# BGI-Qingdao/HAST

Hardware: AMD Instinct MI355X
Metric: classified read-bp/sec at k=21, 150bp reads, 200M unique-mers/hap (higher is better)
Workload: dtype u64; 1 GPU; C3 human-trio scale: 200M+200M synthetic 21-mers, 10M barcodes, 150bp reads; k=21, read_len=150, keys_per_hap=200000000, barcodes=10000000, batch_reads=48000000, reads_total=5760000000, minimizer=16, keys=random, collective=none (D2H of counters in timed region), resident_batches=12

## Files before the change

### hast_amd/binding.py

```python
import ctypes as C
import os
import subprocess

import numpy as np

_HERE = os.path.dirname(os.path.abspath(__file__))
_LIB = None

u8p, u32p, u64p, vp = C.POINTER(C.c_uint8), C.POINTER(C.c_uint32), C.POINTER(C.c_uint64), C.c_void_p

STATUS = {0: "OK", 1: "INVALID", 2: "NO_DEVICE", 3: "HIP", 4: "OOM", 5: "TABLE_FULL", 6: "FORMAT", 7: "RCCL", 8: "IO", 9: "UNSUPPORTED"}


class SynthParams(C.Structure):
    _fields_ = [("seed_k", C.c_uint64), ("seed_r", C.c_uint64), ("seed_b", C.c_uint64),
                ("n_keys_per_hap", C.c_uint64), ("n_barcodes", C.c_uint32), ("read_len", C.c_uint32),
                ("k", C.c_uint32), ("reserved", C.c_uint32)]


class KcSynth(C.Structure):
    _fields_ = [("seed", C.c_uint64), ("genome_len", C.c_uint64), ("read_len", C.c_uint32), ("snp_per_1024", C.c_uint32),
                ("err_per_4096", C.c_uint32), ("n_per_4096", C.c_uint32)]


# ... 64 lines not shown
    "hast_dev_alloc": (C.c_int, [vp, C.c_size_t, C.POINTER(vp)]),
    "hast_dev_free": (C.c_int, [vp, vp]),
    "hast_memcpy_h2d": (C.c_int, [vp, vp, vp, C.c_size_t]),
    "hast_memcpy_d2h": (C.c_int, [vp, vp, vp, C.c_size_t]),
    "hast_memset_d": (C.c_int, [vp, vp, C.c_int, C.c_size_t, vp]),
    "hast_table_reserve": (C.c_int, [vp, C.c_uint64, C.c_double]),
    "hast_table_insert_text": (C.c_int, [vp, C.c_int, C.c_char_p, C.c_size_t, u64p]),
    "hast_table_insert_text_file": (C.c_int, [vp, C.c_int, C.c_char_p, u64p]),
    "hast_ctx_set_text_check": (C.c_int, [vp, C.c_int]),
    "hast_table_insert_keys": (C.c_int, [vp, C.c_int, vp, C.c_size_t]),
    "hast_table_insert_keys_device": (C.c_int, [vp, C.c_int, vp, C.c_size_t, vp]),
    "hast_table_erase": (C.c_int, [vp, vp, C.c_size_t, vp]),
    "hast_table_sizes": (C.c_int, [vp, u64p, u64p]),
    "hast_table_lookup": (C.c_int, [vp, vp, C.c_size_t, vp]),
    "hast_table_save": (C.c_int, [vp, C.c_char_p]),
    "hast_table_load": (C.c_int, [vp, C.c_char_p, C.c_double]),
    "hast_table_file_info": (C.c_int, [C.c_char_p, C.POINTER(C.c_int), u64p]),
    "hast_table_info": (C.c_int, [vp, u64p, u64p]),
    "hast_table_clone": (C.c_int, [vp, vp]),
    "hast_ctx_set_filter": (C.c_int, [vp, C.c_int, C.c_int, C.c_int, C.c_int]),
    "hast_filter_build": (C.c_int, [vp]),
    "hast_filter_info": (C.c_int, [vp, C.POINTER(C.c_int), C.POINTER(C.c_int), C.POINTER(C.c_int), C.POINTER(C.c_int), u64p]),
    "hast_filter_dense": (C.c_int, [vp, C.POINTER(C.c_int)]),
    "hast_filter_request_ceiling": (C.c_int, [vp, C.POINTER(C.c_double)]),
    "hast_counts_resize": (C.c_int, [vp, C.c_size_t]),
    "hast_counts_bind": (C.c_int, [vp, vp, C.c_size_t]),
    "hast_counts_zero": (C.c_int, [vp, vp]),
    "hast_counts_read": (C.c_int, [vp, vp, vp, vp, C.c_size_t]),
    "hast_counts_pack": (C.c_int, [vp, vp, C.c_size_t, vp]),
    "hast_counts_unpack": (C.c_int, [vp, vp, C.c_size_t, vp]),
    "hast_counts_add_votes": (C.c_int, [vp, vp, vp, C.c_size_t, C.c_uint32, vp]),
    "hast_counts_allreduce": (C.c_int, [C.POINTER(vp), C.c_int]),
    "hast_classify_timing": (C.c_int, [vp, C.c_int]),
    "hast_classify_times": (C.c_int, [vp, C.POINTER(C.c_float), C.POINTER(C.c_float), C.c_int, C.POINTER(C.c_int)]),
    "hast_classify_device": (C.c_int, [vp, vp, C.c_size_t, vp, C.c_uint32, vp, vp, C.c_size_t, vp]),
    "hast_classify_batch": (C.c_int, [vp, vp, vp, vp, C.c_size_t, C.c_uint32]),
    "hast_classify_perread_device": (C.c_int, [vp, vp, C.c_size_t, vp, C.c_size_t, vp, vp]),
    "hast_classify_perread": (C.c_int, [vp, vp, vp, C.c_size_t, vp]),
    "hast_batch_begin": (C.c_int, [vp, C.c_size_t, C.c_size_t, C.POINTER(vp), C.POINTER(vp), C.POINTER(vp)]),
    "hast_batch_submit": (C.c_int, [vp, C.c_size_t, C.c_uint32]),
    "hast_names_create": (C.c_int, [vp, C.c_size_t, C.POINTER(vp)]),
    "hast_names_destroy": (None, [vp]),
    "hast_fq_create": (C.c_int, [vp, C.c_size_t, C.c_int, vp, C.POINTER(vp)]),
    "hast_fq_create_ex": (C.c_int, [vp, C.c_size_t, C.c_int, vp, C.c_int, C.POINTER(vp)]),
    "hast_fq_create_striped": (C.c_int, [C.POINTER(vp), C.c_int, C.c_size_t, C.c_int, C.POINTER(vp), C.POINTER(vp)]),
    "hast_fq_create_striped_ex": (C.c_int, [C.POINTER(vp), C.c_int, C.c_size_t, C.c_int, C.POINTER(vp), C.c_int, C.POINTER(vp)]),
# ... 239 lines not shown
    def filter_build(self):
        _ck(self._lib.hast_filter_build(self._h))

    def filter_request_ceiling(self):
        r = C.c_double()
        _ck(self._lib.hast_filter_request_ceiling(self._h, C.byref(r)))
        return r.value

    def filter_info(self):
        en, m, t, kp, b = C.c_int(), C.c_int(), C.c_int(), C.c_int(), C.c_uint64()
        _ck(self._lib.hast_filter_info(self._h, C.byref(en), C.byref(m), C.byref(t), C.byref(kp), C.byref(b)))
        return bool(en.value), m.value, t.value, kp.value, b.value

    def filter_mode(self):
        en = C.c_int()
        _ck(self._lib.hast_filter_info(self._h, C.byref(en), None, None, None, None))
        return en.value

    def filter_dense(self):
        d = C.c_int()
        _ck(self._lib.hast_filter_dense(self._h, C.byref(d)))
        return bool(d.value)

    def close(self):
        if self._h:
            self._lib.hast_ctx_destroy(self._h)
            self._h = C.c_void_p()

    def __enter__(self):
        return self

    def __exit__(self, *a):
        self.close()

    def __del__(self):
        try:
            self.close()
        except Exception:
            pass

    @property
    def stream(self):
        return self._lib.hast_ctx_stream(self._h)

    def sync(self, stream=None):
        _ck(self._lib.hast_stream_sync(self._h, stream))
# ... 499 lines not shown
```

### hast_amd/csrc/classify_main.cpp

```cpp
#include <getopt.h>
#include <sys/stat.h>
#include <unistd.h>

#include <algorithm>
#include <atomic>
#include <cerrno>
#include <chrono>
#include <deque>
#include <cstdarg>
#include <cstdio>
#include <cstdlib>
#include <cstring>
#include <ctime>
#include <condition_variable>
#include <memory>
#include <mutex>
#include <string>
#include <thread>
#include <string_view>
#include <unordered_map>
#include <vector>

#include "../../include/hast.h"
#include "fq_feed.h"
// ... 1771 lines not shown
                (unsigned long long)rs.total_bases, rs.names.size(), rs.t_loaded - rs.t_start, dt, dt > 0 ? rs.total_bases / dt / 1e6 : 0.0);
    }
    if (o.stats && rs.naming.device_dict)
        stat_line("__stats_dictionary__ on=device dictionaries=%zu ids_limit=%zu ids_from_device=%zu ids_from_host=%zu merge_by_text_s=%.3f texts_merged_to_host=%zu rows_summed_by_text=%zu\n", rs.naming.groups.size(), rs.naming.host_base, rs.n_dev_names, rs.n_host_names, rs.naming.merge_s,
                  rs.naming.merged_to_host, rs.n_rows_summed);
    if (o.stats) {
        const char *nc = getenv("HAST_NAME_CACHE"), *rb = getenv("HAST_GZ_RING_BYTES"), *pg = getenv("HAST_PARK_GB");
        stat_line("__stats_sizes__ name_cache=%s gz_ring_bytes=%s park_gb=%s\n", nc ? nc : "default", rb ? rb : "default", pg ? pg : "default");
    }
    if (o.stats) stat_line("__stats_setup__ waited_for_stream_setup_s=%.3f (inside scrub_sizes_clone_s: .gz inputs opened, FASTQ streams created while the table was built)\n", rs.t_pre_waited);
    for (size_t i = 0; i < rs.ctxs.size(); i++) {
        char sw[512] = "";
        (void)hast_ctx_options(rs.ctxs[i], sw, sizeof(sw));
        if (strstr(sw, "filter_fallback"))
            fprintf(stderr, " WARN : GPU %d (context %zu) had no room for the k-mer filter and probed the table directly (%s)\n", o.devices[i], i, sw);
    }
    if (o.stats) {
        char sw[512] = "";
        (void)hast_ctx_options(rs.ctx, sw, sizeof(sw));
        stat_line("__stats_switches__ %s\n", sw[0] ? sw : "none");
        int f_on = 0, f_m = 0, f_t = 0, f_kp = 0;
        uint64_t f_bytes = 0;
        (void)hast_filter_info(rs.ctx, &f_on, &f_m, &f_t, &f_kp, &f_bytes);
        stat_line("__stats_filter__ mode=%s m=%d t=%d kp=%d bytes=%llu\n", f_on == 2 ? "exact_entries" : f_on == 1 ? "prints" : "off_table_only", f_m, f_t, f_kp,
                  (unsigned long long)f_bytes);
    }
    if (rs.hbm_thread.joinable()) {
        rs.hbm_stop = true;
        rs.hbm_thread.join();
        size_t parked = 0;
        (void)hast_dev_mem_info(rs.ctx, nullptr, nullptr, &parked);
        const size_t fm = rs.hbm_free_min.load(), tot = rs.hbm_total.load();
        if (tot) stat_line("__stats_hbm__ total_bytes=%zu free_min_bytes=%zu in_use_peak_bytes=%zu parked_bytes_at_end=%zu\n", tot, fm, tot - std::min(fm, tot), parked);
    }
    fprintf(stderr, "__END__\n");
    rs.t_printed = now_s();
}

int leave(Run &rs) {
    const Options &o = rs.o;
    const char *preload = getenv("LD_PRELOAD");
    const bool profiled = getenv("ROCP_TOOL_LIBRARIES") || (preload && strstr(preload, "rocprofiler"));
    if (!getenv("HAST_TEARDOWN") && !profiled) {
        if (o.stats) stat_phases(rs, nullptr);
        if (!o.stats_json.empty() && !write_stats_json(o.stats_json)) fprintf(stderr, "classify: cannot write %s\n", o.stats_json.c_str());
        if (fflush(stdout) != 0) die_output();
        fflush(stderr);
        _exit(0);
// ... 51 lines not shown
```

### hast_amd/csrc/hast_api.cpp

```cpp
#include <dlfcn.h>
#include <fcntl.h>
#include <sys/stat.h>
#include <unistd.h>
#include <hip/hip_runtime.h>

#include <algorithm>
#include <chrono>
#include <atomic>
#include <cstdarg>
#include <cstdio>
#include <cstdlib>
#include <cstring>
#include <functional>
#include <map>
#include <mutex>
#include <new>
#include <string>
#include <vector>

#include "../../include/hast.h"
#include "hast_common.h"
#include "hast_device.h"
#include "kc_device.h"
#include "fq_device.h"
// ... 271 lines not shown
        else c->exact_env_off = atoi(e) == 0;
    }
    if (c->exact_env_off) c->filter_exact = 0;
    else if (c->exact_env_once) c->filter_exact = 1;
    if (const char *e = getenv("HAST_COMMIT")) c->commit_mode = !strcmp(e, "atomic") ? 1 : !strcmp(e, "partition") ? 2 : 0;
    if (const char *e = getenv("HAST_PART_SPAN")) c->part_span = (uint32_t)atoi(e);
    if (const char *e = getenv("HAST_F_GEO")) c->kernel_geo = e[0] != '0';
    if (const char *e = getenv("HAST_F_RL")) c->kernel_rl = e[0] != '0';
    if (const char *e = getenv("HAST_TILE_LDS")) {
        const long v = atol(e);
        if (v >= 4096 && v <= 160 * 1024) c->tile_lds = (size_t)v;
    }
    hipDeviceProp_t prop;
    if (hipGetDeviceProperties(&prop, device) == hipSuccess) c->n_cu = prop.multiProcessorCount;
    tr("hipGetDeviceProperties");
    hast_status st = HAST_OK;
    auto bail = [&](hipError_t he, const char *what) {
        if (he != hipSuccess && st == HAST_OK) st = set_error(HAST_ERR_HIP, "%s: %s", what, hipGetErrorString(he));
    };
    bail(hipStreamCreateWithFlags(&c->stream, hipStreamNonBlocking), "hipStreamCreate");
    tr("hipStreamCreate");
    bail(dev_malloc(&c->d_err, 4 * sizeof(uint32_t)), "dev_malloc(err)");
    tr("first hipMalloc");
    bail(dev_malloc(&c->d_cnt, 8 * sizeof(unsigned long long)), "dev_malloc(cnt)");
    bail(pinned_malloc(reinterpret_cast<void **>(&c->h_errword), 64, hipHostMallocDefault), "pinned_malloc(err word)");
    if (st == HAST_OK) bail(hipMemsetAsync(c->d_err, 0, 4 * sizeof(uint32_t), c->stream), "hipMemset");
    if (st == HAST_OK) bail(hipStreamSynchronize(c->stream), "hipStreamSynchronize");
    tr("first fill + synchronize");
    for (auto &s : c->stage)
        if (st == HAST_OK) bail(hipEventCreateWithFlags(&s.done, hipEventDisableTiming), "hipEventCreate");
    tr("events");
    if (st != HAST_OK) {
        hast_ctx_destroy(c);
        return st;
    }
    *out = c;
    return HAST_OK;
}

void hast_release_parked(void) { release_parked(); }

void hast_ctx_destroy(hast_ctx *c) {
    if (!c) return;
    (void)hipSetDevice(c->device);
    if (c->stream) (void)hipStreamSynchronize(c->stream);
    release_parked();
    for (auto &s : c->stage) {
// ... 404 lines not shown
    dst->nbuckets = 0;
    dst->filter_valid = false;
    dst->m = src->m;
    const size_t bytes = table_slots(src) * sizeof(uint64_t);
    HAST_HIP_TRY(dev_malloc(&dst->d_slots, bytes));
    HAST_HIP_TRY(hipMemcpyPeerAsync(dst->d_slots, dst->device, src->d_slots, src->device, bytes, dst->stream));
    dst->nbuckets = src->nbuckets;
    if (src->filter_valid && dst->use_filter) {
        if (dst->filter_bytes != src->filter_bytes) {
            if (dst->d_filter) HAST_HIP_TRY(hipFree(dst->d_filter));
            dst->d_filter = nullptr;
            dst->filter_bytes = 0;
            if (dst->test_filter_oom || dev_malloc(&dst->d_filter, src->filter_bytes) != hipSuccess) {
                (void)hipGetLastError();
                dst->d_filter = nullptr;
                dst->use_filter = false;
                dst->filter_fallback_bytes = src->filter_bytes;
                HAST_HIP_TRY(hipStreamSynchronize(dst->stream));
                return HAST_OK;
            }
            dst->filter_bytes = src->filter_bytes;
        }
        HAST_HIP_TRY(hipMemcpyPeerAsync(dst->d_filter, dst->device, src->d_filter, src->device, src->filter_bytes, dst->stream));
        dst->fg = src->fg;
        dst->filter_m = src->filter_m;
        dst->filter_exact = src->filter_exact;
        dst->filter_t = src->filter_t;
        dst->filter_kp = src->filter_kp;
        dst->filter_valid = true;
    }
    HAST_HIP_TRY(hipStreamSynchronize(dst->stream));
    return HAST_OK;
}

hast_status hast_table_info(const hast_ctx *c, uint64_t *n_buckets, uint64_t *bytes) {
    if (!c) return set_error(HAST_ERR_INVALID, "null context");
    if (n_buckets) *n_buckets = c->nbuckets;
    if (bytes) *bytes = (uint64_t)table_slots(c) * sizeof(uint64_t);
    return HAST_OK;
}

hast_status hast_counts_resize(hast_ctx *c, size_t n) {
    if (hast_status st = use(c)) return st;
    HAST_HIP_TRY(hipStreamSynchronize(c->stream));
    if (c->counts_owned && c->d_counts) HAST_HIP_TRY(hipFree(c->d_counts));
    c->d_counts = nullptr;
// ... 199 lines not shown
    FilterGeom fg = filter_geom_for(c->k, h[0] + h[1], c->filter_m, c->filter_t, c->filter_kp, c->k == 32 ? 0 : c->filter_exact);
    size_t bytes = (size_t)filter_nblocks(fg) * 128;
    if (bytes != c->filter_bytes) {
        if (c->d_filter) HAST_HIP_TRY(hipFree(c->d_filter));
        c->d_filter = nullptr;
        c->filter_bytes = 0;
        hipError_t got = c->test_filter_oom ? hipErrorOutOfMemory : dev_malloc(&c->d_filter, bytes);
        if (got != hipSuccess && !c->filter_m && fg.m == kFilterMaxM) {
            (void)hipGetLastError();
            fg = filter_geom_for(c->k, h[0] + h[1], kFilterMaxM - 1, c->filter_t, c->filter_kp, c->k == 32 ? 0 : c->filter_exact);
            bytes = (size_t)filter_nblocks(fg) * 128;
            got = dev_malloc(&c->d_filter, bytes);
        }
        if (got != hipSuccess) {
            (void)hipGetLastError();
            c->d_filter = nullptr;
            c->use_filter = false;
            c->filter_fallback_bytes = bytes;
            return HAST_OK;
        }
        c->filter_bytes = bytes;
    }
    HAST_HIP_TRY(hipMemsetAsync(c->d_filter, 0, bytes, hs));
    HAST_HIP_TRY(launch_filter_build(c->d_slots, geom(c), c->d_filter, fg, hs));
    c->fg = fg;
    c->filter_valid = true;
    return HAST_OK;
}

static constexpr uint32_t kSegWindows = 482;
static constexpr uint32_t kLongRead = 4096;

static hast_status commit_prepare(hast_ctx *c, size_t n_reads, uint32_t max_votes, bool atomic_only, hipStream_t hs, commit::Plan *pl, bool *partitioned) {
    *partitioned = false;
    const int mode = c->commit_mode;
    if (mode == 1 || atomic_only || c->part_oom) return HAST_OK;
    *pl = commit::plan_for(n_reads, c->n_barcodes, c->part_span);
    if (!commit::usable(*pl, n_reads, max_votes, mode == 2)) return HAST_OK;
    if (c->part.bytes < pl->bytes) {
        HAST_HIP_TRY(hipStreamSynchronize(hs));
        if (c->part.d) HAST_HIP_TRY(hipFree(c->part.d));
        c->part = CommitScratch{};
        if (dev_malloc(&c->part.d, pl->bytes + pl->bytes / 8) == hipSuccess) c->part.bytes = pl->bytes + pl->bytes / 8;
        else {
            (void)hipGetLastError();
            c->part.d = nullptr;
            c->part_oom = true;
// ... 192 lines not shown
    if (hast_status st = need_table(c, 0)) return st;
    if (!c->use_filter) return HAST_OK;
    if (hast_status st = ensure_filter(c, c->stream)) return st;
    HAST_HIP_TRY(hipStreamSynchronize(c->stream));
    return HAST_OK;
}

hast_status hast_filter_info(const hast_ctx *c, int *enabled, int *m, int *t, int *kp, uint64_t *bytes) {
    if (!c) return set_error(HAST_ERR_INVALID, "null context");
    if (enabled) *enabled = !c->use_filter ? 0 : (c->filter_valid && c->fg.exact) ? 2 : 1;
    if (m) *m = c->filter_valid ? c->fg.m : 0;
    if (t) *t = c->filter_valid ? c->fg.t : 0;
    if (kp) *kp = c->filter_valid ? c->fg.kp : 0;
    if (bytes) *bytes = c->filter_valid ? c->filter_bytes : 0;
    return HAST_OK;
}

hast_status hast_filter_dense(const hast_ctx *c, int *dense) {
    if (!c || !dense) return set_error(HAST_ERR_INVALID, "null argument");
    *dense = (c->use_filter && c->filter_valid && c->fg.dense) ? 1 : 0;
    return HAST_OK;
}

hast_status hast_filter_request_ceiling(hast_ctx *c, double *requests_per_s) {
    if (hast_status st = need_table(c, 0)) return st;
    if (!requests_per_s) return set_error(HAST_ERR_INVALID, "null argument");
    if (!c->use_filter) return set_error(HAST_ERR_INVALID, "the filter is off");
    if (hast_status st = ensure_filter(c, c->stream)) return st;
    if (!c->use_filter || !c->d_filter) return set_error(HAST_ERR_INVALID, "no filter (HBM too small for it)");
    const uint64_t nblocks = filter_nblocks(c->fg);
    const int grid = c->n_cu * 8;
    const uint32_t iters = 256;
    uint32_t *d_sink = reinterpret_cast<uint32_t *>(c->d_cnt + 2);
    hipEvent_t e0 = nullptr, e1 = nullptr;
    hipError_t e = hipEventCreate(&e0);
    if (e == hipSuccess) e = hipEventCreate(&e1);
    float best = 0;
    for (int rep = 0; rep < 3 && e == hipSuccess; ++rep) {
        e = hipEventRecord(e0, c->stream);
        if (e == hipSuccess) e = launch_request_ceiling(c->d_filter, nblocks, iters, grid, d_sink, c->stream);
        if (e == hipSuccess) e = hipEventRecord(e1, c->stream);
        if (e == hipSuccess) e = hipEventSynchronize(e1);
        float ms = 0;
        if (e == hipSuccess) e = hipEventElapsedTime(&ms, e0, e1);
        if (e == hipSuccess && rep && (best == 0 || ms < best)) best = ms;
    }
// ... 335 lines not shown
```

### hast_amd/csrc/hast_common.h

```cpp
#pragma once
#include <stdint.h>

#include "tmer_level_table.h"

#if defined(__HIPCC__)
#include <hip/hip_runtime.h>
#define HAST_HD __host__ __device__ __forceinline__
#else
#define HAST_HD inline
#endif

namespace hast {

HAST_HD uint32_t base_code(uint32_t c) { return (c & 6u) >> 1; }
HAST_HD uint64_t kmer_mask(int k) { return k >= 32 ? ~0ull : (1ull << (2 * k)) - 1; }

HAST_HD uint64_t kmer_revcomp(uint64_t x, int k) {
    x ^= 0xAAAAAAAAAAAAAAAAull;
#if defined(__HIP_DEVICE_COMPILE__)
    x = __brevll(x);
    x = ((x & 0x5555555555555555ull) << 1) | ((x >> 1) & 0x5555555555555555ull);
#else
    x = ((x & 0x3333333333333333ull) << 2) | ((x >> 2) & 0x3333333333333333ull);
    x = ((x & 0x0F0F0F0F0F0F0F0Full) << 4) | ((x >> 4) & 0x0F0F0F0F0F0F0F0Full);
// ... 132 lines not shown
    return h ^ (h >> 15);
}
HAST_HD uint32_t filter_sub_of(uint32_t keyhash) { return keyhash >> 29; }
HAST_HD uint32_t filter_sub2_of(uint32_t keyhash) { return (keyhash >> 26) & 7u; }
HAST_HD uint32_t filter_print_of(uint32_t keyhash) {
    const uint32_t f = (keyhash >> 8) & 0xFFFFu;
    return f ? f : 1u;
}
HAST_HD int filter_pos_bits(const FilterGeom &g) {
    int b = 0;
    while ((1u << b) < filter_w(g)) ++b;
    return b;
}
HAST_HD bool filter_exact_fits(const FilterGeom &g) { return g.k <= 32 && g.m <= 14 && 2 * (g.k - g.m) + filter_pos_bits(g) <= 17; }
HAST_HD uint32_t filter_exact_code(uint64_t fwd, uint32_t pm, const FilterGeom &g) {
    const int rb = 2 * (g.k - g.m);
    const uint32_t rest = ((uint32_t)fwd << (2 * pm)) | (uint32_t)(fwd >> (2 * ((uint32_t)g.k - pm)));
    const uint32_t code = (rest & ((1u << rb) - 1u)) | (pm << rb);
    return mul24_forced(code, 0x1D2C5u) & 0x1FFFFu;
}
HAST_HD uint32_t filter_exact_sub(uint32_t code17) { return code17 >> 14; }
HAST_HD uint32_t filter_exact_entry(uint32_t code17, uint32_t tags) { return ((code17 & 0x3FFFu) << 2) | tags; }
constexpr uint32_t kFilterOverflowMark = 0xFFFCu;
constexpr double kFilterDenseMaxLoad = 3.2;
HAST_HD uint32_t filter_dense_pm(uint32_t p, uint32_t w) { return (w - 1u - p) & (w - 1u); }
HAST_HD double filter_dense_load(const FilterGeom &g, uint64_t n_keys) {
    return 2.0 * (double)filter_w(g) * (double)n_keys / ((double)kFilterSubs * (double)filter_nblocks(g));
}
HAST_HD FilterGeom filter_geom_for(int k, uint64_t n_keys, int m_override, int t_override, int kp_override = 0, int exact_mode = -1) {
    FilterGeom g;
    g.k = k;
    int m = k < 8 ? k : 8;
    while (m < k && m < kFilterMaxM && (1ull << (2 * m)) * 3 < 2 * n_keys) ++m;
    if (exact_mode && n_keys >= (16ull << 20) && k - 7 > m && k - 7 <= 14) m = k - 7;
    while (m < kFilterMaxM && k >= m + 9 && 2.0 * (double)n_keys > 2.2 * (double)(1ull << (2 * m))) ++m;
    if (m_override >= 1 && m_override <= k && m_override <= kFilterMaxM) m = m_override;
    g.m = m;
    int kp = k < m + 8 ? k : m + 8;
    if (kp_override >= m && kp_override <= k && kp_override - m < 32) kp = kp_override;
    g.kp = kp;
    const int w = kp - m + 1, r = m < 4 ? m : 4;
    int t = r + (m - r) % w;
    if (t_override >= 1 && t_override <= m) t = t_override;
    g.t = t;
    const int nt = kp - t + 1;
    g.g = nt < 4 ? nt : 4;
// ... 84 lines not shown
```

### hast_amd/csrc/hast_device.h

```cpp
#pragma once
#include <hip/hip_runtime.h>
#include <stddef.h>
#include <stdint.h>
#include "commit_plan.h"
#include "hast_common.h"

namespace hast {

struct TableGeom {
    uint32_t nbuckets;
    int k;
    int m;
    int wide;
};

struct ClassifyArgs {
    const uint8_t *bases;
    uint64_t bases_bytes;
    const uint64_t *offsets;
    const uint32_t *lens;
    const uint32_t *seg_read;
    uint32_t *votes;
    uint16_t *votes16;
    unsigned long long *tile_queue;
// ... 9 lines not shown
    uint32_t mh_stride;
    uint32_t div_mh;
    uint32_t div_hw;
    int k;
    int m;
    int wide;
    int strict;
    const void *filter;
    FilterGeom fg;
    uint32_t l1_stride;
    uint32_t div_l1g;
};

hipError_t launch_insert_keys(uint64_t *slots, TableGeom g, const uint64_t *d_keys, size_t n, uint32_t hap,
                              uint32_t *d_err, hipStream_t s);
hipError_t launch_insert_text(uint64_t *slots, TableGeom g, const char *d_text, size_t n_lines,
                              uint32_t hap, int acgt_only, uint32_t *d_err, hipStream_t s);
hipError_t launch_erase_keys(uint64_t *slots, TableGeom g, const uint64_t *d_keys, size_t n, uint8_t *d_hit, hipStream_t s);
hipError_t launch_lookup_keys(uint64_t *slots, TableGeom g, const uint64_t *d_keys, size_t n, uint8_t *d_tags, hipStream_t s);
hipError_t launch_export_slots(const uint64_t *slots, size_t nslots, uint64_t *d_out, size_t cap, unsigned long long *d_counter, hipStream_t s);
hipError_t launch_import_slots(uint64_t *slots, TableGeom g, const uint64_t *d_in, size_t n, uint32_t *d_err, hipStream_t s);
hipError_t launch_count_tags(const uint64_t *slots, TableGeom g, unsigned long long *d_out, hipStream_t s);
hipError_t launch_classify(const ClassifyArgs &a, int grid, size_t smem, hipStream_t s);
hipError_t launch_filter_build(const uint64_t *slots, TableGeom g, void *filter, FilterGeom fg, hipStream_t s);
hipError_t launch_classify_f(const ClassifyArgs &a, int grid, size_t smem, int variants, hipStream_t s);
hipError_t launch_request_ceiling(const void *filter, uint64_t nblocks, uint32_t iters, int grid, uint32_t *d_sink, hipStream_t s);
size_t classify_f_queue_bytes();
hipError_t launch_build_segments(const uint64_t *d_offsets, const uint32_t *d_lens, uint64_t fixed_len, size_t n_reads, int k, uint32_t seg_windows, uint64_t *seg_off,
                                 uint32_t *seg_len, uint32_t *seg_read, unsigned long long *d_counter, const uint8_t *d_skip,
                                 uint64_t cap, uint64_t bases_bytes, uint32_t *d_err, hipStream_t s);
hipError_t launch_scan_n(const uint8_t *d_bases, const uint64_t *d_offsets, const uint32_t *d_lens, uint64_t fixed_len, size_t n_reads, uint8_t *d_has_n, hipStream_t s);
hipError_t launch_commit_votes(const uint32_t *d_votes, const uint32_t *d_barcode_ids, unsigned long long *d_counts, uint32_t *d_votes_out,
                               size_t n_reads, hipStream_t s);
struct CommitScratch {
    void *d = nullptr;
    size_t bytes = 0;
    uint32_t n_bins = 0, cap = 0;
    uint32_t parity = 0;
};
hipError_t launch_commit_partitioned(const void *d_votes, bool votes16, const uint32_t *d_barcode_ids, unsigned long long *d_counts, size_t n_barcodes,
                                     size_t n_reads, const commit::Plan &pl, CommitScratch &sc, hipStream_t s);
hipError_t launch_add_u64(unsigned long long *d_dst, const unsigned long long *d_src, size_t n, hipStream_t s);
hipError_t launch_counts_pack(const unsigned long long *d_counts, unsigned long long *d_packed, size_t n, hipStream_t s);
hipError_t launch_counts_unpack(unsigned long long *d_counts, const unsigned long long *d_packed, size_t n, hipStream_t s);
hipError_t launch_synth_keys(const SynthParams &p, int hap, uint64_t first, size_t n, uint64_t *d_out, hipStream_t s);
hipError_t launch_synth_reads(const SynthParams &p, uint64_t first, size_t n, uint8_t *d_bases, uint32_t *d_bc, hipStream_t s);

// ... 2 lines not shown
```

### hast_amd/csrc/hast_filter.hip

```cpp
#include "hast_common.h"
#include "hast_device.h"
#include "hast_devutil.h"

namespace hast {

__device__ __forceinline__ uint32_t sub_load(const uint32_t *w) {
    uint32_t n = 0;
    for (int i = 0; i < kFilterPrints / 2; ++i) {
        const uint32_t v = __hip_atomic_load(&w[i], __ATOMIC_RELAXED, __HIP_MEMORY_SCOPE_AGENT);
        n += (v & 0xFFFFu) != 0;
        n += (v >> 16) != 0;
    }
    return n;
}
__device__ __forceinline__ bool sub_insert(uint32_t *w, uint32_t fp) {
    for (int i = 0; i < kFilterPrints / 2;) {
        const uint32_t v = __hip_atomic_load(&w[i], __ATOMIC_RELAXED, __HIP_MEMORY_SCOPE_AGENT);
        const uint32_t lo = v & 0xFFFFu, hi = v >> 16;
        if (lo == fp || hi == fp) return true;
        uint32_t nv;
        if (lo == 0) nv = v | fp;
        else if (hi == 0) nv = v | (fp << 16);
        else { ++i; continue; }
        if (atomicCAS(&w[i], v, nv) == v) return true;
    }
    return false;
}
__device__ __forceinline__ void sub_mark_overflow(uint32_t *w) {
    uint32_t v = __hip_atomic_load(&w[kFilterPrints / 2 - 1], __ATOMIC_RELAXED, __HIP_MEMORY_SCOPE_AGENT);
    while ((v >> 16) != kFilterOverflowMark) {
        const uint32_t old = atomicCAS(&w[kFilterPrints / 2 - 1], v, (v & 0xFFFFu) | (kFilterOverflowMark << 16));
        if (old == v) break;
        v = old;
    }
}
__device__ __forceinline__ void filter_insert(uint32_t *filt, const FilterGeom g, uint64_t key, uint32_t tags) {
    for (int o = 0; o < 2; ++o) {
        const uint64_t s = o ? kmer_revcomp(key, g.k) : key;
        if (o && s == key) break;
        if (g.exact) {
            const uint32_t pm0 = g.dense ? 0u : filter_sample_pos(s, g), pm1 = g.dense ? filter_w(g) : pm0 + 1u;
            for (uint32_t pm = pm0; pm < pm1; ++pm) {
                const uint32_t blk = filter_block_of((uint32_t)(s >> (2 * (g.k - g.m - (int)pm))) & (uint32_t)kmer_mask(g.m), g.m);
                const uint32_t c17 = filter_exact_code(s, pm, g);
                uint32_t *w = filt + (size_t)blk * (kFilterSubs * kFilterPrints / 2) + filter_exact_sub(c17) * (kFilterPrints / 2);
                if (!sub_insert(w, filter_exact_entry(c17, tags))) sub_mark_overflow(w);
            }
            continue;
        }
        const uint32_t blk = filter_block_of_string(s, g);
        const uint32_t h = filter_keyhash(s), fp = filter_print_of(h);
        uint32_t *b = filt + (size_t)blk * (kFilterSubs * kFilterPrints / 2);
        uint32_t *w1 = b + filter_sub_of(h) * (kFilterPrints / 2), *w2 = b + filter_sub2_of(h) * (kFilterPrints / 2);
        if (g.choices == 1) {
            (void)sub_insert(w1, fp);
            continue;
        }
        bool there = false;
        for (int i = 0; i < kFilterPrints / 2 && !there; ++i) {
            const uint32_t v = __hip_atomic_load(&w2[i], __ATOMIC_RELAXED, __HIP_MEMORY_SCOPE_AGENT);
            there = (v & 0xFFFFu) == fp || (v >> 16) == fp;
        }
        if (there) continue;
        if (w1 != w2 && sub_load(w2) < sub_load(w1)) { uint32_t *t = w1; w1 = w2; w2 = t; }
        if (!sub_insert(w1, fp) && w1 != w2) (void)sub_insert(w2, fp);
    }
}

__global__ void __launch_bounds__(256) k_filter_build(const uint64_t *slots, size_t nslots, uint32_t *filt, FilterGeom g, int wide) {
    for (size_t i = blockIdx.x * (size_t)blockDim.x + threadIdx.x; i < nslots; i += (size_t)gridDim.x * blockDim.x) {
        const uint64_t s = slots[i];
        if (wide) {
            if (s < kTombSlot) filter_insert(filt, g, s, 0);
        } else if (s != kEmptySlot && (s & 3)) filter_insert(filt, g, s >> 2, (uint32_t)(s & 3));
    }
}

hipError_t launch_filter_build(const uint64_t *slots, TableGeom tg, void *filter, FilterGeom fg, hipStream_t s) {
    const size_t nslots = (size_t)tg.nbuckets * kSlotsPerBucket * (tg.wide ? 2 : 1);
    size_t grid = (nslots + 255) / 256;
    if (grid > 256 * 32) grid = 256 * 32;
    hipLaunchKernelGGL(k_filter_build, dim3((unsigned)grid), dim3(256), 0, s, slots, nslots, (uint32_t *)filter, fg, tg.wide);
    return hipGetLastError();
}

constexpr int kThreadsF = 256;
constexpr int kQCap = 128;
#ifndef HAST_F_MINWAVES
#define HAST_F_MINWAVES 5
#endif
#ifndef HAST_F_MINWAVES_DENSE
#define HAST_F_MINWAVES_DENSE 5
#endif
typedef unsigned long long u64x2f __attribute__((ext_vector_type(2)));
typedef unsigned int u32x4f __attribute__((ext_vector_type(4)));
typedef unsigned short u16x2f __attribute__((ext_vector_type(2)));

size_t classify_f_queue_bytes() { return (size_t)4 * kQCap * 3 * sizeof(uint32_t); }

__device__ __forceinline__ uint32_t pk_min_u16(uint32_t a, uint32_t b) {
    const u16x2f r = __builtin_elementwise_min(__builtin_bit_cast(u16x2f, a), __builtin_bit_cast(u16x2f, b));
    return __builtin_bit_cast(uint32_t, r);
}
__device__ __forceinline__ unsigned long long ballot64(bool p) { return __builtin_amdgcn_ballot_w64(p); }
__device__ __forceinline__ uint32_t pk_max_u16(uint32_t a, uint32_t b) {
// ... 253 lines not shown
            uint32_t pm;
            if (DENSE) {
                pm = filter_dense_pm(p, W);
            } else {
                const uint32_t *l1 = s_l1 + mul24(r, L1S) + p;
                uint32_t x = l1[0];
                if (NTC) {
#pragma unroll
                    for (int c = 1; c + 1 < (NTC ? NTC : 1); ++c) x = min(x, l1[c * 4]);
                } else {
                    for (uint32_t c = 1; c + 1 < ntc; ++c) x = min(x, l1[c * G]);
                }
                if (ntc > 1) x = min(x, l1[NT - G]);
                const uint32_t xr = ((x & 0xFFFu) - p) & 63u;
                pm = (GEO && (W & (W - 1)) == 0) ? (xr & (W - 1)) : xr - mul24(mul24(xr, fg.wdiv) >> 16, W);
            }
            const uint32_t mm = (uint32_t)(fwd >> (2 * ((uint32_t)(K - M) - pm))) & mmask;
            uint32_t fb = ok ? filter_block_of(mm, M) : 0xFFFFFFFFu;
            const uint32_t h = EXACT ? filter_exact_code(fwd, pm, fg) : filter_keyhash(fwd);
            const uint32_t anchor = okm ? (uint32_t)__builtin_amdgcn_readlane((int)fb, (int)__builtin_ctzll(okm)) : last_fb;
            last_fb = anchor;
            fb = ok ? fb : anchor;
            if (EXACT) {
                B.v = filt[(fb << 3) | filter_exact_sub(h)];
                B.fpw = mul24((h & 0x3FFFu) ^ 0x3FFFu, 0x00040004u);
            } else {
                B.v = filt[(size_t)fb * kFilterSubs + filter_sub_of(h)];
                if (TWO) B.v2 = filt[(size_t)fb * kFilterSubs + filter_sub2_of(h)];
                const uint32_t fp = filter_print_of(h);
                B.fpw = fp | (fp << 16);
            }
            B.klo = (uint32_t)fwd;
            B.khi = (uint32_t)(fwd >> 32);
            B.meta = r | (ok ? 0x80000000u : 0u);
            pos = pos + 64 < q_end ? pos + 64 : q_end;
            if (P >= 64) {
                cp += 64;
                const bool wrap = cp >= P;
                cp -= wrap ? P : 0u;
                cr += wrap ? 1u : 0u;
            } else locate();
        };
        auto finish = [&](Blk &B) {
            bool pos;
            if (EXACT) {
                const uint32_t mx = pk_max_u16(pk_max_u16(B.v.x ^ B.fpw, B.v.y ^ B.fpw), pk_max_u16(B.v.z ^ B.fpw, B.v.w ^ B.fpw));
                const uint32_t m16 = max(mx >> 16, mx & 0xFFFFu);
                const bool valid = (int)B.meta < 0;
                const bool hit = valid && m16 >= 0xFFFDu;
                if (hit) atomicAdd(&s_vote[B.meta & 0xFFFFu], (unsigned long long)(m16 & 1u) | ((unsigned long long)((m16 >> 1) & 1u) << 32));
                pos = valid && !hit && (B.v.w >> 16) == kFilterOverflowMark;
            } else {
            uint32_t acc = pk_min_u16(pk_min_u16(B.v.x ^ B.fpw, B.v.y ^ B.fpw), pk_min_u16(B.v.z ^ B.fpw, B.v.w ^ B.fpw));
            bool full = (B.v.w >> 16) != 0;
            if (TWO) {
                acc = pk_min_u16(acc, pk_min_u16(pk_min_u16(B.v2.x ^ B.fpw, B.v2.y ^ B.fpw), pk_min_u16(B.v2.z ^ B.fpw, B.v2.w ^ B.fpw)));
                full = full && (B.v2.w >> 16) != 0;
            }
            const bool match = ((acc - 0x00010001u) & ~acc & 0x80008000u) != 0;
            pos = (int)B.meta < 0 && (match || full);
            }
            const unsigned long long pmask = ballot64(pos);
            if (pmask) {
                const uint32_t at = qn + lanes_below(pmask);
                if (pos) {
                    q_lo[at] = B.klo;
                    q_hi[at] = B.khi;
                    q_rd[at] = B.meta & 0xFFFFu;
                }
                qn += (uint32_t)__popcll(pmask);
                if (qn >= 64) drain(64);
            }
        };
        {
// ... 130 lines not shown
```

### include/hast.h

```cpp
#ifndef HAST_H
#define HAST_H
#include <stddef.h>
#include <stdint.h>

#ifdef __cplusplus
extern "C" {
#endif

typedef enum {
    HAST_OK = 0,
    HAST_ERR_INVALID = 1,
    HAST_ERR_NO_DEVICE = 2,
    HAST_ERR_HIP = 3,
    HAST_ERR_OOM = 4,
    HAST_ERR_TABLE_FULL = 5,
    HAST_ERR_FORMAT = 6,
    HAST_ERR_RCCL = 7,
    HAST_ERR_IO = 8,
    HAST_ERR_UNSUPPORTED = 9
} hast_status;

typedef struct hast_ctx hast_ctx;
typedef void *hast_stream;

// ... 28 lines not shown
hast_status hast_ctx_set_text_check(hast_ctx *, int acgt_only);
hast_status hast_table_insert_keys(hast_ctx *, int hap, const uint64_t *canon_keys, size_t n);
hast_status hast_table_insert_keys_device(hast_ctx *, int hap, const uint64_t *d_canon_keys, size_t n,
                                          hast_stream);

hast_status hast_table_erase(hast_ctx *, const uint64_t *canon_keys, size_t n, uint8_t *out_hit);

hast_status hast_table_sizes(hast_ctx *, uint64_t *n_hap0, uint64_t *n_hap1);

hast_status hast_table_lookup(hast_ctx *, const uint64_t *canon_keys, size_t n, uint8_t *out_tags);

hast_status hast_table_save(hast_ctx *, const char *path);
hast_status hast_table_load(hast_ctx *, const char *path, double load_factor);
hast_status hast_table_file_info(const char *path, int *k_out, uint64_t *n_keys_out);

hast_status hast_table_clone(hast_ctx *dst, hast_ctx *src);

hast_status hast_table_info(const hast_ctx *, uint64_t *n_buckets, uint64_t *bytes);

hast_status hast_ctx_set_filter(hast_ctx *, int enable, int m, int t, int kp);
hast_status hast_filter_build(hast_ctx *);
hast_status hast_filter_info(const hast_ctx *, int *enabled, int *m, int *t, int *kp, uint64_t *bytes);
hast_status hast_filter_dense(const hast_ctx *, int *dense);
hast_status hast_filter_request_ceiling(hast_ctx *, double *requests_per_s);

hast_status hast_counts_resize(hast_ctx *, size_t n_barcodes);
hast_status hast_counts_bind(hast_ctx *, uint64_t *d_counts, size_t n_barcodes);
hast_status hast_counts_zero(hast_ctx *, hast_stream);
hast_status hast_counts_read(hast_ctx *, uint64_t *c0, uint64_t *c1, uint64_t *neg, size_t n_barcodes);
hast_status hast_counts_read_range(hast_ctx *, size_t first, size_t n, uint64_t *c0, uint64_t *c1, uint64_t *neg);
hast_status hast_counts_pack(hast_ctx *, uint64_t *d_packed, size_t n_barcodes, hast_stream);
hast_status hast_counts_unpack(hast_ctx *, const uint64_t *d_packed, size_t n_barcodes, hast_stream);
hast_status hast_counts_add_votes(hast_ctx *, const uint32_t *d_votes, const uint32_t *d_barcode_ids, size_t n_reads,
                                  uint32_t max_votes, hast_stream);
hast_status hast_counts_allreduce(hast_ctx *const *ctxs, int n_ctx);
hast_status hast_counts_permute(hast_ctx *, const uint32_t *perm, size_t n_perm, size_t n_new);

hast_status hast_classify_device(hast_ctx *, const uint8_t *d_bases, size_t bases_bytes,
                                 const uint64_t *d_offsets, uint32_t read_len,
                                 const uint32_t *d_barcode_ids, uint32_t *d_votes,
                                 size_t n_reads, hast_stream);
hast_status hast_classify_timing(hast_ctx *, int n_slots);
hast_status hast_classify_times(hast_ctx *, float *classify_ms, float *commit_ms, int max, int *n_out);
hast_status hast_classify_batch(hast_ctx *, const uint8_t *bases, const uint64_t *offsets,
                                const uint32_t *barcode_ids, size_t n_reads, uint32_t max_read_len);

// ... 238 lines not shown
```

Measured before the change: 385.6 billion bp/s.

## Lodge overflowed exact-filter entries as guests in sibling sub-buckets

Exact-filter sub-buckets that overflow now get a soft mark, and a second build pass stores the overflowed entries as guests in the sibling sub-bucket. A hard overflow mark is set only when the sibling has no room either. The classify kernel loads the sibling sub-bucket as well and checks it when the soft mark is set, so fewer k-mers fall back to probing the hash table. The cost is an extra 16-byte filter load per lookup, an extra build kernel, and a small set of counters exposed through a new stats API.

```diff
diff --git a/hast_amd/binding.py b/hast_amd/binding.py
--- a/hast_amd/binding.py
+++ b/hast_amd/binding.py
@@ -110,6 +110,7 @@
     "hast_filter_build": (C.c_int, [vp]),
     "hast_filter_info": (C.c_int, [vp, C.POINTER(C.c_int), C.POINTER(C.c_int), C.POINTER(C.c_int), C.POINTER(C.c_int), u64p]),
     "hast_filter_dense": (C.c_int, [vp, C.POINTER(C.c_int)]),
+    "hast_filter_marks": (C.c_int, [vp, u64p]),
     "hast_filter_request_ceiling": (C.c_int, [vp, C.POINTER(C.c_double)]),
     "hast_counts_resize": (C.c_int, [vp, C.c_size_t]),
     "hast_counts_bind": (C.c_int, [vp, vp, C.c_size_t]),
@@ -395,6 +396,11 @@
         _ck(self._lib.hast_filter_dense(self._h, C.byref(d)))
         return bool(d.value)
 
+    def filter_marks(self):
+        out = (C.c_uint64 * 4)()
+        _ck(self._lib.hast_filter_marks(self._h, out))
+        return tuple(int(x) for x in out)
+
     def close(self):
         if self._h:
             self._lib.hast_ctx_destroy(self._h)
diff --git a/hast_amd/csrc/classify_main.cpp b/hast_amd/csrc/classify_main.cpp
--- a/hast_amd/csrc/classify_main.cpp
+++ b/hast_amd/csrc/classify_main.cpp
@@ -1817,8 +1817,11 @@
         int f_on = 0, f_m = 0, f_t = 0, f_kp = 0;
         uint64_t f_bytes = 0;
         (void)hast_filter_info(rs.ctx, &f_on, &f_m, &f_t, &f_kp, &f_bytes);
-        stat_line("__stats_filter__ mode=%s m=%d t=%d kp=%d bytes=%llu\n", f_on == 2 ? "exact_entries" : f_on == 1 ? "prints" : "off_table_only", f_m, f_t, f_kp,
-                  (unsigned long long)f_bytes);
+        uint64_t f_marks[4] = {0, 0, 0, 0};
+        (void)hast_filter_marks(rs.ctx, f_marks);
+        stat_line("__stats_filter__ mode=%s m=%d t=%d kp=%d bytes=%llu soft_marks=%llu hard_marks=%llu guests=%llu without_room=%llu\n",
+                  f_on == 2 ? "exact_entries" : f_on == 1 ? "prints" : "off_table_only", f_m, f_t, f_kp, (unsigned long long)f_bytes,
+                  (unsigned long long)f_marks[0], (unsigned long long)f_marks[1], (unsigned long long)f_marks[2], (unsigned long long)f_marks[3]);
     }
     if (rs.hbm_thread.joinable()) {
         rs.hbm_stop = true;
diff --git a/hast_amd/csrc/filter_build_core.h b/hast_amd/csrc/filter_build_core.h
--- /dev/null
+++ b/hast_amd/csrc/filter_build_core.h
@@ -0,0 +1,81 @@
+#pragma once
+#include "hast_common.h"
+
+namespace hast {
+namespace fb {
+
+constexpr int kWords = kFilterPrints / 2;
+constexpr int kBlockWords = kFilterSubs * kWords;
+enum Counter { kMarksSet = 0, kMarksHard = 1, kGuests = 2, kNoRoom = 3, kCounters = 4 };
+
+
+template <class A> HAST_HD int sub_insert(A &a, uint32_t *w, uint32_t e) {
+    for (int i = 0; i < kWords;) {
+        const uint32_t v = a.load(&w[i]);
+        const uint32_t lo = v & 0xFFFFu, hi = v >> 16;
+        if (lo == e || hi == e) return 1;
+        uint32_t nv;
+        if (lo == 0) nv = v | e;
+        else if (hi == 0) nv = v | (e << 16);
+        else { ++i; continue; }
+        if (a.cas(&w[i], v, nv) == v) return 2;
+    }
+    return 0;
+}
+template <class A> HAST_HD bool sub_mark(A &a, uint32_t *w, uint32_t mark) {
+    uint32_t v = a.load(&w[kWords - 1]);
+    while ((v >> 16) != mark && (v >> 16) != kFilterOverflowMark) {
+        const uint32_t old = a.cas(&w[kWords - 1], v, (v & 0xFFFFu) | (mark << 16));
+        if (old == v) return true;
+        v = old;
+    }
+    return false;
+}
+HAST_HD uint32_t *sub_words(uint32_t *filt, uint32_t blk, uint32_t sub) { return filt + (size_t)blk * kBlockWords + sub * kWords; }
+
+template <class A> HAST_HD void file_native(A &a, uint32_t *filt, uint32_t blk, uint32_t c17, uint32_t tags) {
+    uint32_t *w = sub_words(filt, blk, filter_exact_sub(c17));
+    if (!fb::sub_insert(a, w, filter_exact_entry(c17, tags)) && fb::sub_mark(a, w, kFilterSoftMark)) a.count(kMarksSet);
+}
+template <class A> HAST_HD void lodge_guest(A &a, uint32_t *filt, uint32_t blk, uint32_t c17, uint32_t tags) {
+    uint32_t *w = sub_words(filt, blk, filter_exact_sub(c17));
+    const uint32_t last = a.load(&w[kWords - 1]);
+    if (!filter_is_mark(last >> 16)) return;
+    const uint32_t e = filter_exact_entry(c17, tags);
+    if ((last & 0xFFFFu) == e) return;
+    for (int i = 0; i < kWords - 1; ++i) {
+        const uint32_t v = a.load(&w[i]);
+        if ((v & 0xFFFFu) == e || (v >> 16) == e) return;
+    }
+    if (filter_guest_storable(c17)) {
+        const int r = fb::sub_insert(a, fb::sub_words(filt, blk, filter_guest_sub(c17)), filter_guest_entry(c17));
+        if (r == 2) a.count(kGuests);
+        if (r) return;
+    }
+    a.count(kNoRoom);
+    if (fb::sub_mark(a, w, kFilterOverflowMark)) a.count(kMarksHard);
+}
+
+template <class F> HAST_HD void for_each_filing(const FilterGeom &g, uint64_t key, F f) {
+    for (int o = 0; o < 2; ++o) {
+        const uint64_t s = o ? kmer_revcomp(key, g.k) : key;
+        if (o && s == key) break;
+        const uint32_t pm0 = g.dense ? 0u : filter_sample_pos(s, g), pm1 = g.dense ? filter_w(g) : pm0 + 1u;
+        for (uint32_t pm = pm0; pm < pm1; ++pm)
+            f(filter_block_of((uint32_t)(s >> (2 * (g.k - g.m - (int)pm))) & (uint32_t)kmer_mask(g.m), g.m), filter_exact_code(s, pm, g));
+    }
+}
+
+struct PlainWords {
+    uint64_t n[kCounters] = {0, 0, 0, 0};
+    uint32_t load(const uint32_t *p) { return *p; }
+    uint32_t cas(uint32_t *p, uint32_t expected, uint32_t desired) {
+        const uint32_t old = *p;
+        if (old == expected) *p = desired;
+        return old;
+    }
+    void count(int c) { ++n[c]; }
+};
+
+}
+}
diff --git a/hast_amd/csrc/hast_api.cpp b/hast_amd/csrc/hast_api.cpp
--- a/hast_amd/csrc/hast_api.cpp
+++ b/hast_amd/csrc/hast_api.cpp
@@ -317,7 +317,7 @@
     tr("hipStreamCreate");
     bail(dev_malloc(&c->d_err, 4 * sizeof(uint32_t)), "dev_malloc(err)");
     tr("first hipMalloc");
-    bail(dev_malloc(&c->d_cnt, 8 * sizeof(unsigned long long)), "dev_malloc(cnt)");
+    bail(dev_malloc(&c->d_cnt, 12 * sizeof(unsigned long long)), "dev_malloc(cnt)");
     bail(pinned_malloc(reinterpret_cast<void **>(&c->h_errword), 64, hipHostMallocDefault), "pinned_malloc(err word)");
     if (st == HAST_OK) bail(hipMemsetAsync(c->d_err, 0, 4 * sizeof(uint32_t), c->stream), "hipMemset");
     if (st == HAST_OK) bail(hipStreamSynchronize(c->stream), "hipStreamSynchronize");
@@ -768,6 +768,7 @@
             dst->filter_bytes = src->filter_bytes;
         }
         HAST_HIP_TRY(hipMemcpyPeerAsync(dst->d_filter, dst->device, src->d_filter, src->device, src->filter_bytes, dst->stream));
+        HAST_HIP_TRY(hipMemcpyPeerAsync(dst->d_cnt + 8, dst->device, src->d_cnt + 8, src->device, 4 * sizeof(unsigned long long), dst->stream));
         dst->fg = src->fg;
         dst->filter_m = src->filter_m;
         dst->filter_exact = src->filter_exact;
@@ -1013,7 +1014,7 @@
         c->filter_bytes = bytes;
     }
     HAST_HIP_TRY(hipMemsetAsync(c->d_filter, 0, bytes, hs));
-    HAST_HIP_TRY(launch_filter_build(c->d_slots, geom(c), c->d_filter, fg, hs));
+    HAST_HIP_TRY(launch_filter_build(c->d_slots, geom(c), c->d_filter, fg, c->d_cnt + 8, hs));
     c->fg = fg;
     c->filter_valid = true;
     return HAST_OK;
@@ -1252,6 +1253,21 @@
     return HAST_OK;
 }
 
+hast_status hast_filter_marks(hast_ctx *c, uint64_t out[4]) {
+    if (!c || !out) return set_error(HAST_ERR_INVALID, "null argument");
+    for (int i = 0; i < 4; ++i) out[i] = 0;
+    if (!c->use_filter || !c->filter_valid || !c->d_filter) return HAST_OK;
+    if (hast_status st = use(c)) return st;
+    unsigned long long h[4] = {0, 0, 0, 0};
+    HAST_HIP_TRY(hipMemcpyAsync(h, c->d_cnt + 8, sizeof(h), hipMemcpyDeviceToHost, c->stream));
+    HAST_HIP_TRY(hipStreamSynchronize(c->stream));
+    out[0] = h[0] - h[1];
+    out[1] = h[1];
+    out[2] = h[2];
+    out[3] = h[3];
+    return HAST_OK;
+}
+
 hast_status hast_filter_request_ceiling(hast_ctx *c, double *requests_per_s) {
     if (hast_status st = need_table(c, 0)) return st;
     if (!requests_per_s) return set_error(HAST_ERR_INVALID, "null argument");
diff --git a/hast_amd/csrc/hast_common.h b/hast_amd/csrc/hast_common.h
--- a/hast_amd/csrc/hast_common.h
+++ b/hast_amd/csrc/hast_common.h
@@ -178,6 +178,11 @@
 HAST_HD uint32_t filter_exact_sub(uint32_t code17) { return code17 >> 14; }
 HAST_HD uint32_t filter_exact_entry(uint32_t code17, uint32_t tags) { return ((code17 & 0x3FFFu) << 2) | tags; }
 constexpr uint32_t kFilterOverflowMark = 0xFFFCu;
+constexpr uint32_t kFilterSoftMark = 0xFFF8u;
+HAST_HD bool filter_is_mark(uint32_t e) { return e == kFilterSoftMark || e == kFilterOverflowMark; }
+HAST_HD bool filter_guest_storable(uint32_t code17) { const uint32_t c = code17 & 0x3FFFu; return c != 0u && c < 0x3FFEu; }
+HAST_HD uint32_t filter_guest_entry(uint32_t code17) { return (code17 & 0x3FFFu) << 2; }
+HAST_HD uint32_t filter_guest_sub(uint32_t code17) { return filter_exact_sub(code17) ^ 1u; }
 constexpr double kFilterDenseMaxLoad = 3.2;
 HAST_HD uint32_t filter_dense_pm(uint32_t p, uint32_t w) { return (w - 1u - p) & (w - 1u); }
 HAST_HD double filter_dense_load(const FilterGeom &g, uint64_t n_keys) {
diff --git a/hast_amd/csrc/hast_device.h b/hast_amd/csrc/hast_device.h
--- a/hast_amd/csrc/hast_device.h
+++ b/hast_amd/csrc/hast_device.h
@@ -55,7 +55,7 @@
 hipError_t launch_import_slots(uint64_t *slots, TableGeom g, const uint64_t *d_in, size_t n, uint32_t *d_err, hipStream_t s);
 hipError_t launch_count_tags(const uint64_t *slots, TableGeom g, unsigned long long *d_out, hipStream_t s);
 hipError_t launch_classify(const ClassifyArgs &a, int grid, size_t smem, hipStream_t s);
-hipError_t launch_filter_build(const uint64_t *slots, TableGeom g, void *filter, FilterGeom fg, hipStream_t s);
+hipError_t launch_filter_build(const uint64_t *slots, TableGeom g, void *filter, FilterGeom fg, unsigned long long *marks, hipStream_t s);
 hipError_t launch_classify_f(const ClassifyArgs &a, int grid, size_t smem, int variants, hipStream_t s);
 hipError_t launch_request_ceiling(const void *filter, uint64_t nblocks, uint32_t iters, int grid, uint32_t *d_sink, hipStream_t s);
 size_t classify_f_queue_bytes();
diff --git a/hast_amd/csrc/hast_filter.hip b/hast_amd/csrc/hast_filter.hip
--- a/hast_amd/csrc/hast_filter.hip
+++ b/hast_amd/csrc/hast_filter.hip
@@ -1,9 +1,16 @@
 #include "hast_common.h"
 #include "hast_device.h"
 #include "hast_devutil.h"
+#include "filter_build_core.h"
 
 namespace hast {
 
+struct AtomicWords {
+    unsigned long long *n;
+    __device__ __forceinline__ uint32_t load(const uint32_t *p) { return __hip_atomic_load(p, __ATOMIC_RELAXED, __HIP_MEMORY_SCOPE_AGENT); }
+    __device__ __forceinline__ uint32_t cas(uint32_t *p, uint32_t expected, uint32_t desired) { return atomicCAS(p, expected, desired); }
+    __device__ __forceinline__ void count(int c) { atomicAdd(&n[c], 1ull); }
+};
 __device__ __forceinline__ uint32_t sub_load(const uint32_t *w) {
     uint32_t n = 0;
     for (int i = 0; i < kFilterPrints / 2; ++i) {
@@ -13,47 +20,21 @@
     }
     return n;
 }
-__device__ __forceinline__ bool sub_insert(uint32_t *w, uint32_t fp) {
-    for (int i = 0; i < kFilterPrints / 2;) {
-        const uint32_t v = __hip_atomic_load(&w[i], __ATOMIC_RELAXED, __HIP_MEMORY_SCOPE_AGENT);
-        const uint32_t lo = v & 0xFFFFu, hi = v >> 16;
-        if (lo == fp || hi == fp) return true;
-        uint32_t nv;
-        if (lo == 0) nv = v | fp;
-        else if (hi == 0) nv = v | (fp << 16);
-        else { ++i; continue; }
-        if (atomicCAS(&w[i], v, nv) == v) return true;
-    }
-    return false;
-}
-__device__ __forceinline__ void sub_mark_overflow(uint32_t *w) {
-    uint32_t v = __hip_atomic_load(&w[kFilterPrints / 2 - 1], __ATOMIC_RELAXED, __HIP_MEMORY_SCOPE_AGENT);
-    while ((v >> 16) != kFilterOverflowMark) {
-        const uint32_t old = atomicCAS(&w[kFilterPrints / 2 - 1], v, (v & 0xFFFFu) | (kFilterOverflowMark << 16));
-        if (old == v) break;
-        v = old;
-    }
-}
-__device__ __forceinline__ void filter_insert(uint32_t *filt, const FilterGeom g, uint64_t key, uint32_t tags) {
+__device__ __forceinline__ bool print_insert(AtomicWords &aw, uint32_t *w, uint32_t fp) { return fb::sub_insert(aw, w, fp) != 0; }
+__device__ __forceinline__ void filter_insert(AtomicWords &aw, uint32_t *filt, const FilterGeom g, uint64_t key, uint32_t tags) {
+    if (g.exact) {
+        fb::for_each_filing(g, key, [&](uint32_t blk, uint32_t c17) { fb::file_native(aw, filt, blk, c17, tags); });
+        return;
+    }
     for (int o = 0; o < 2; ++o) {
         const uint64_t s = o ? kmer_revcomp(key, g.k) : key;
         if (o && s == key) break;
-        if (g.exact) {
-            const uint32_t pm0 = g.dense ? 0u : filter_sample_pos(s, g), pm1 = g.dense ? filter_w(g) : pm0 + 1u;
-            for (uint32_t pm = pm0; pm < pm1; ++pm) {
-                const uint32_t blk = filter_block_of((uint32_t)(s >> (2 * (g.k - g.m - (int)pm))) & (uint32_t)kmer_mask(g.m), g.m);
-                const uint32_t c17 = filter_exact_code(s, pm, g);
-                uint32_t *w = filt + (size_t)blk * (kFilterSubs * kFilterPrints / 2) + filter_exact_sub(c17) * (kFilterPrints / 2);
-                if (!sub_insert(w, filter_exact_entry(c17, tags))) sub_mark_overflow(w);
-            }
-            continue;
-        }
         const uint32_t blk = filter_block_of_string(s, g);
         const uint32_t h = filter_keyhash(s), fp = filter_print_of(h);
         uint32_t *b = filt + (size_t)blk * (kFilterSubs * kFilterPrints / 2);
         uint32_t *w1 = b + filter_sub_of(h) * (kFilterPrints / 2), *w2 = b + filter_sub2_of(h) * (kFilterPrints / 2);
         if (g.choices == 1) {
-            (void)sub_insert(w1, fp);
+            (void)print_insert(aw, w1, fp);
             continue;
         }
         bool there = false;
@@ -63,24 +44,38 @@
         }
         if (there) continue;
         if (w1 != w2 && sub_load(w2) < sub_load(w1)) { uint32_t *t = w1; w1 = w2; w2 = t; }
-        if (!sub_insert(w1, fp) && w1 != w2) (void)sub_insert(w2, fp);
-    }
-}
-
-__global__ void __launch_bounds__(256) k_filter_build(const uint64_t *slots, size_t nslots, uint32_t *filt, FilterGeom g, int wide) {
+        if (!print_insert(aw, w1, fp) && w1 != w2) (void)print_insert(aw, w2, fp);
+    }
+}
+
+__global__ void __launch_bounds__(256) k_filter_build(const uint64_t *slots, size_t nslots, uint32_t *filt, FilterGeom g, int wide, unsigned long long *marks) {
+    AtomicWords aw{marks};
     for (size_t i = blockIdx.x * (size_t)blockDim.x + threadIdx.x; i < nslots; i += (size_t)gridDim.x * blockDim.x) {
         const uint64_t s = slots[i];
         if (wide) {
-            if (s < kTombSlot) filter_insert(filt, g, s, 0);
-        } else if (s != kEmptySlot && (s & 3)) filter_insert(filt, g, s >> 2, (uint32_t)(s & 3));
-    }
-}
-
-hipError_t launch_filter_build(const uint64_t *slots, TableGeom tg, void *filter, FilterGeom fg, hipStream_t s) {
+            if (s < kTombSlot) filter_insert(aw, filt, g, s, 0);
+        } else if (s != kEmptySlot && (s & 3)) filter_insert(aw, filt, g, s >> 2, (uint32_t)(s & 3));
+    }
+}
+__global__ void __launch_bounds__(256) k_filter_guests(const uint64_t *slots, size_t nslots, uint32_t *filt, FilterGeom g, unsigned long long *marks) {
+    if (marks[fb::kMarksSet] == 0) return;
+    AtomicWords aw{marks};
+    for (size_t i = blockIdx.x * (size_t)blockDim.x + threadIdx.x; i < nslots; i += (size_t)gridDim.x * blockDim.x) {
+        const uint64_t s = slots[i];
+        if (s == kEmptySlot || !(s & 3)) continue;
+        const uint32_t tags = (uint32_t)(s & 3);
+        fb::for_each_filing(g, s >> 2, [&](uint32_t blk, uint32_t c17) { fb::lodge_guest(aw, filt, blk, c17, tags); });
+    }
+}
+
+hipError_t launch_filter_build(const uint64_t *slots, TableGeom tg, void *filter, FilterGeom fg, unsigned long long *marks, hipStream_t s) {
     const size_t nslots = (size_t)tg.nbuckets * kSlotsPerBucket * (tg.wide ? 2 : 1);
     size_t grid = (nslots + 255) / 256;
     if (grid > 256 * 32) grid = 256 * 32;
-    hipLaunchKernelGGL(k_filter_build, dim3((unsigned)grid), dim3(256), 0, s, slots, nslots, (uint32_t *)filter, fg, tg.wide);
+    hipError_t e = hipMemsetAsync(marks, 0, fb::kCounters * sizeof(unsigned long long), s);
+    if (e != hipSuccess) return e;
+    hipLaunchKernelGGL(k_filter_build, dim3((unsigned)grid), dim3(256), 0, s, slots, nslots, (uint32_t *)filter, fg, tg.wide, marks);
+    if (fg.exact && !tg.wide) hipLaunchKernelGGL(k_filter_guests, dim3((unsigned)grid), dim3(256), 0, s, slots, nslots, (uint32_t *)filter, fg, marks);
     return hipGetLastError();
 }
 
@@ -380,7 +375,9 @@
             last_fb = anchor;
             fb = ok ? fb : anchor;
             if (EXACT) {
-                B.v = filt[(fb << 3) | filter_exact_sub(h)];
+                const uint32_t sb = (fb << 3) | filter_exact_sub(h);
+                B.v = filt[sb];
+                B.v2 = filt[sb ^ 1u];
                 B.fpw = mul24((h & 0x3FFFu) ^ 0x3FFFu, 0x00040004u);
             } else {
                 B.v = filt[(size_t)fb * kFilterSubs + filter_sub_of(h)];
@@ -407,7 +404,14 @@
                 const bool valid = (int)B.meta < 0;
                 const bool hit = valid && m16 >= 0xFFFDu;
                 if (hit) atomicAdd(&s_vote[B.meta & 0xFFFFu], (unsigned long long)(m16 & 1u) | ((unsigned long long)((m16 >> 1) & 1u) << 32));
-                pos = valid && !hit && (B.v.w >> 16) == kFilterOverflowMark;
+                const uint32_t s7 = B.v.w >> 16;
+                pos = valid && !hit && s7 == kFilterOverflowMark;
+                const bool soft = valid && !hit && s7 == kFilterSoftMark;
+                if (ballot64(soft)) {
+                    const uint32_t gw = B.fpw ^ 0xFFFCFFFCu;
+                    const uint32_t acc = pk_min_u16(pk_min_u16(B.v2.x ^ gw, B.v2.y ^ gw), pk_min_u16(B.v2.z ^ gw, B.v2.w ^ gw));
+                    pos = pos || (soft && ((acc - 0x00010001u) & ~acc & 0x80008000u) != 0);
+                }
             } else {
             uint32_t acc = pk_min_u16(pk_min_u16(B.v.x ^ B.fpw, B.v.y ^ B.fpw), pk_min_u16(B.v.z ^ B.fpw, B.v.w ^ B.fpw));
             bool full = (B.v.w >> 16) != 0;
diff --git a/include/hast.h b/include/hast.h
--- a/include/hast.h
+++ b/include/hast.h
@@ -74,6 +74,7 @@
 hast_status hast_filter_build(hast_ctx *);
 hast_status hast_filter_info(const hast_ctx *, int *enabled, int *m, int *t, int *kp, uint64_t *bytes);
 hast_status hast_filter_dense(const hast_ctx *, int *dense);
+hast_status hast_filter_marks(hast_ctx *, uint64_t out[4]);
 hast_status hast_filter_request_ceiling(hast_ctx *, double *requests_per_s);
 
 hast_status hast_counts_resize(hast_ctx *, size_t n_barcodes);
```

Result: no change. 385.9 billion bp/s, median of 6 (+0.1%).
